# gusanagy/Hybrid-Diffusion-Underwater-Atmopheric-Image-Enhancement

Hardware: AMD Instinct MI355X
Metric: denoising-steps/sec (256x256, T=1000) (higher is better)
Workload: dtype f32 (tensors and accumulation fp32; every operand of the attention contractions as 2xfp16 pieces -- scores: a balance per product term, four terms at d_head 16 / three at d_head 32; P.V: three terms -- and of the 3x3 convs behind GroupNorm likewise (other 3x3 convs: 3xbf16 pieces), on the 16-bit MFM

## Files before the change

### hybrid-diffusion-underwater-atmopheric-image-enhancement_amd/csrc/conv1x1_x3.hip

```cpp
#include <stdlib.h>

#include "common.h"
#include "conv_x3.h"
#include "device.h"

using namespace hdiff;

namespace {

constexpr int THREADS = 256;

__device__ constexpr int TERM_W[6] = {2, 1, 0, 1, 0, 0};
__device__ constexpr int TERM_X[6] = {0, 1, 2, 0, 1, 0};

template <bool WLDS>
__global__ __launch_bounds__(THREADS, 3) void conv1x1_x3_kernel(const Conv1x1X3K p) {
  constexpr int MT = 2, WN = 2;
  __shared__ __attribute__((aligned(16))) u32x4 sW[WLDS ? 2 : 1][WLDS ? 3 * 64 * 2 : 1];
  const int tid = threadIdx.x, lane = tid & 63, wave = tid >> 6;
  const int l31 = lane & 31, h = lane >> 5;
  int cob = blockIdx.x, tile_id = blockIdx.y;
  if ((gridDim.y & 7u) == 0u && gridDim.x > 1u) {
    const unsigned lin = blockIdx.x + gridDim.x * blockIdx.y, per = 8u * gridDim.x;
    const unsigned grp = lin / per, r = lin - grp * per;
    tile_id = (int)(grp * 8u + (r & 7u));
    cob = (int)(r >> 3);
  }
  const int co0 = cob * 64;
  const long px0 = ((long)tile_id * 4 + __builtin_amdgcn_readfirstlane(wave)) * 64;
  const int b = blockIdx.z;
  const int C1 = p.Cin - p.C0;
  const unsigned hw = (unsigned)p.HW;
  const float* x0b = p.x0 + (size_t)b * p.C0 * p.HW + px0;
  const float* x1b = p.x1 ? p.x1 + (size_t)b * C1 * p.HW + px0 - (size_t)p.C0 * p.HW : x0b;
  const unsigned* wlane = p.wp3 + ((size_t)(co0 + l31) * 8 + h * 4);
  const size_t w_piece = (size_t)p.CoutPad * 8, w_chunk = 3 * w_piece;

  f32x16 acc[MT][WN];
#pragma unroll
  for (int mt = 0; mt < MT; ++mt)
#pragma unroll
    for (int nt = 0; nt < WN; ++nt)
#pragma unroll
      for (int r = 0; r < 16; ++r) acc[mt][nt][r] = 0.f;

  constexpr int XD = 1;
  const int nchunks = p.Cin / 16;
  f32x2 xr[XD + 1][8];
  u32x4 wr[2][MT][3];
  auto load_x = [&](f32x2 (&x)[8], int c) {
    c = min(c, nchunks - 1);
    const float* xb = (16 * c < p.C0) ? x0b : x1b;
    const unsigned k0 = (unsigned)(16 * c + 8 * h);
#pragma unroll
    for (int j = 0; j < 8; ++j) x[j] = *reinterpret_cast<const f32x2*>(xb + (size_t)((k0 + j) * hw + 2u * l31));
  };
  auto load_w = [&](u32x4 (&w)[MT][3], int c) {
    const unsigned* wb = wlane + (size_t)min(c, nchunks - 1) * w_chunk;
#pragma unroll
    for (int mt = 0; mt < MT; ++mt)
#pragma unroll
      for (int pc = 0; pc < 3; ++pc) w[mt][pc] = *reinterpret_cast<const u32x4*>(wb + pc * w_piece + (size_t)mt * 32 * 8);
  };
  auto mma = [&](const f32x2 (&x)[8], const u32x4 (&w)[MT][3]) {
    u32x4 xp[WN][3];
#pragma unroll
    for (int nt = 0; nt < WN; ++nt)
#pragma unroll
      for (int j = 0; j < 4; ++j) {
        unsigned h0, h1, h2;
        split3(x[2 * j][nt], x[2 * j + 1][nt], h0, h1, h2);
        xp[nt][0][j] = h0; xp[nt][1][j] = h1; xp[nt][2][j] = h2;
      }
#pragma unroll
    for (int t = 0; t < 6; ++t) {
      if ((HDIFF_MUTANT & 1) && TERM_W[t] == 0 && TERM_X[t] == 2) continue;
#pragma unroll
      for (int mt = 0; mt < MT; ++mt)
#pragma unroll
        for (int nt = 0; nt < WN; ++nt) acc[mt][nt] = mfma_bf16(w[mt][TERM_W[t]], xp[nt][TERM_X[t]], acc[mt][nt]);
    }
  };

  if constexpr (WLDS) {
    const unsigned* wsrc[2];
    int wdst[2];
#pragma unroll
    for (int i = 0; i < 2; ++i) {
      int u = i * THREADS + tid;
      if (u >= 384) u -= 128;
      const int pc = u >> 7, rem = u & 127;
      wsrc[i] = p.wp3 + (size_t)pc * w_piece + (size_t)(co0 + (rem >> 1)) * 8 + (rem & 1) * 4;
      wdst[i] = u;
    }
    u32x4 wst[2];
    auto wload = [&](int c) {
      const size_t off = (size_t)min(c, nchunks - 1) * w_chunk;
#pragma unroll
      for (int i = 0; i < 2; ++i) wst[i] = *reinterpret_cast<const u32x4*>(wsrc[i] + off);
    };
    auto wstore = [&](int buf) {
#pragma unroll
      for (int i = 0; i < 2; ++i) sW[buf][wdst[i]] = wst[i];
    };
    auto wread = [&](u32x4 (&w)[MT][3], int buf) {
#pragma unroll
      for (int mt = 0; mt < MT; ++mt)
#pragma unroll
        for (int pc = 0; pc < 3; ++pc) w[mt][pc] = sW[buf][(pc * 64 + 32 * mt + l31) * 2 + h];
    };
    wload(0);
    load_x(xr[0], 0);
    wstore(0);
    __syncthreads();
    for (int c = 0; c < nchunks; c += 2) {
#pragma unroll
      for (int i = 0; i < 2; ++i) {
        if (c + i < nchunks) {
          wload(c + i + 1);
          load_x(xr[(i + 1) & 1], c + i + 1);
          wread(wr[0], i);
          mma(xr[i], wr[0]);
          wstore((i + 1) & 1);
          asm volatile("s_waitcnt lgkmcnt(0)\n\ts_barrier" ::: "memory");
        }
      }
    }
  } else {
#pragma unroll
    for (int i = 0; i < XD; ++i) load_x(xr[i], i);
    load_w(wr[0], 0);
    for (int c = 0; c < nchunks; c += XD + 1) {
#pragma unroll
      for (int i = 0; i < XD + 1; ++i) {
        if (c + i < nchunks) {
          load_x(xr[(i + XD) % (XD + 1)], c + i + XD);
          load_w(wr[(i + 1) & 1], c + i + 1);
          mma(xr[i], wr[i & 1]);
        }
      }
    }
  }

  const size_t blk = ((size_t)b * p.Cout) * p.HW + px0;
  const bool full = co0 + 64 <= p.Cout;
  const bool track = p.absmax_out != nullptr;
  unsigned amax = 0u;
#pragma unroll
  for (int mt = 0; mt < MT; ++mt) {
#pragma unroll
    for (int r0 = 0; r0 < 16; r0 += 8) {
      f32x2 res[8];
      float add[8];
      bool ok[8];
#pragma unroll
      for (int j = 0; j < 8; ++j) {
        const int r = r0 + j;
        const int co = co0 + 32 * mt + (r & 3) + 8 * (r >> 2) + 4 * h;
        ok[j] = full || co < p.Cout;
        const int cc = ok[j] ? co : 0;
        float a = 0.f;
        if (p.bias) a += p.bias[cc];
        if (p.addvec) a += p.addvec[(size_t)b * p.Cout + cc];
        add[j] = a;
        if (p.residual) res[j] = *reinterpret_cast<const f32x2*>(p.residual + blk + (size_t)cc * p.HW + 2u * l31);
      }
#pragma unroll
      for (int j = 0; j < 8; ++j) {
        const int r = r0 + j;
        const int co = co0 + 32 * mt + (r & 3) + 8 * (r >> 2) + 4 * h;
        f32x2 v = {acc[mt][0][r], acc[mt][1][r]};
        v += add[j];
        if (p.residual) v += res[j];
        if (ok[j]) *reinterpret_cast<f32x2*>(p.out + blk + (size_t)co * p.HW + 2u * l31) = v;
        if (track && ok[j]) {
          const unsigned v0 = __builtin_bit_cast(unsigned, v[0]) & 0x7fffffffu, v1 = __builtin_bit_cast(unsigned, v[1]) & 0x7fffffffu;
          const unsigned vm = v0 > v1 ? v0 : v1;
          amax = vm > amax ? vm : amax;
        }
      }
    }
  }
  if (track) {
#pragma unroll
    for (int o = 32; o > 0; o >>= 1) {
      const unsigned other = (unsigned)__shfl_xor((int)amax, o, 64);
      amax = other > amax ? other : amax;
    }
    if (lane == 0) atomicMax(&p.absmax_out[b], amax);
  }
}

}

namespace hdiff {

void launch_conv1x1_x3(const Conv1x1X3K& k, int B, hipStream_t stream) {
  dim3 grid(cdiv(k.Cout, 64), (unsigned)(k.HW / 256), B);
  hipLaunchKernelGGL(conv1x1_x3_kernel<true>, grid, dim3(THREADS), 0, stream, k);
}

}
```

Baseline: 3.018.

## Add persistent LDS-resident-weight kernel for 1x1 x3 convolution

Adds a persistent kernel variant where each workgroup loads the whole 3-piece weight slice for its 64 output channels into LDS once, then loops over pixel tiles with cross-tile prefetch of the next input chunk and next bias/addvec. This is meant to remove repeated per-tile weight streaming and LDS double-buffer barriers, and to amortise launch and tail cost by sizing the grid to the device's CU count with XCD-aware slot mapping. It relies on large dynamic LDS (up to 160KB) and falls back to the old kernel when that cannot be set or occupancy would be poor.

Measured after the change: 3.024, median of 2. Within noise of the previous version (+0.2%).

```diff
diff --git a/hybrid-diffusion-underwater-atmopheric-image-enhancement_amd/csrc/conv1x1_x3.hip b/hybrid-diffusion-underwater-atmopheric-image-enhancement_amd/csrc/conv1x1_x3.hip
--- a/hybrid-diffusion-underwater-atmopheric-image-enhancement_amd/csrc/conv1x1_x3.hip
+++ b/hybrid-diffusion-underwater-atmopheric-image-enhancement_amd/csrc/conv1x1_x3.hip
@@ -1,4 +1,6 @@
 #include <stdlib.h>
+
+#include <atomic>
 
 #include "common.h"
 #include "conv_x3.h"
@@ -191,12 +193,237 @@
   }
 }
 
+#ifndef CONV1X1_RESIDENT
+#define CONV1X1_RESIDENT 1
+#endif
+constexpr int res_wps(bool res) { return res ? 2 : 3; }
+template <int NW, bool RES>
+__global__ __launch_bounds__(NW * 64, res_wps(RES)) void conv1x1_x3_resident_kernel(const Conv1x1X3K p, const int B, const int nslots) {
+  constexpr int MT = 2, WN = 2, NT = NW * 64;
+  extern __shared__ __attribute__((aligned(16))) u32x4 sWr[];
+  const int tid = threadIdx.x, lane = tid & 63, wave = __builtin_amdgcn_readfirstlane(tid >> 6);
+  const int l31 = lane & 31, h = lane >> 5;
+  const unsigned per = 8u * (gridDim.x / (unsigned)nslots);
+  const unsigned grp = blockIdx.x / per, r = blockIdx.x - grp * per;
+  const int slot = (int)(grp * 8u + (r & 7u)), co0_wg = (int)(r >> 3) * 64;
+  const int tps = (int)(p.HW >> 6), ntiles = B * tps, tstep = nslots * NW;
+  if (slot * NW >= ntiles) return;
+  const int C1 = p.Cin - p.C0;
+  const unsigned hw = (unsigned)p.HW;
+  const int nchunks = p.Cin / 16;
+  const size_t w_piece = (size_t)p.CoutPad * 8, w_chunk = 3 * w_piece;
+
+  const int nunits = nchunks * 384;
+  for (int u0 = tid; u0 < nunits; u0 += 4 * NT) {
+    u32x4 v[4];
+#pragma unroll
+    for (int i = 0; i < 4; ++i) {
+      const int u = min(u0 + i * NT, nunits - 1);
+      const int c = u / 384, q = u - c * 384, pc = q >> 7, rem = q & 127;
+      v[i] = *reinterpret_cast<const u32x4*>(p.wp3 + (size_t)c * w_chunk + (size_t)pc * w_piece + (size_t)(co0_wg + (rem >> 1)) * 8 + (rem & 1) * 4);
+    }
+#pragma unroll
+    for (int i = 0; i < 4; ++i)
+      if (u0 + i * NT < nunits) sWr[u0 + i * NT] = v[i];
+  }
+  __syncthreads();
+
+  struct Tile { const float* x0; const float* x1; int b; long px0; };
+  auto tile_at = [&](int t) {
+    const int b = t / tps;
+    const long px0 = (long)(t - b * tps) * 64;
+    const float* x0 = p.x0 + (size_t)b * p.C0 * p.HW + px0;
+    return Tile{x0, p.x1 ? p.x1 + (size_t)b * C1 * p.HW + px0 - (size_t)p.C0 * p.HW : x0, b, px0};
+  };
+  auto load_x = [&](f32x2 (&x)[8], const float* x0, const float* x1, int c) {
+    const float* xb = (16 * c < p.C0) ? x0 : x1;
+    const unsigned k0 = (unsigned)(16 * c + 8 * h);
+#pragma unroll
+    for (int j = 0; j < 8; ++j) x[j] = *reinterpret_cast<const f32x2*>(xb + (size_t)((k0 + j) * hw + 2u * l31));
+  };
+  f32x16 acc[MT][WN];
+  auto mma = [&](const f32x2 (&x)[8], int c) {
+    u32x4 w[MT][3];
+#pragma unroll
+    for (int mt = 0; mt < MT; ++mt)
+#pragma unroll
+      for (int pc = 0; pc < 3; ++pc) w[mt][pc] = sWr[c * 384 + (pc * 64 + 32 * mt + l31) * 2 + h];
+    u32x4 xp[WN][3];
+#pragma unroll
+    for (int nt = 0; nt < WN; ++nt)
+#pragma unroll
+      for (int j = 0; j < 4; ++j) {
+        unsigned h0, h1, h2;
+        split3(x[2 * j][nt], x[2 * j + 1][nt], h0, h1, h2);
+        xp[nt][0][j] = h0; xp[nt][1][j] = h1; xp[nt][2][j] = h2;
+      }
+#pragma unroll
+    for (int t = 0; t < 6; ++t) {
+      if ((HDIFF_MUTANT & 1) && TERM_W[t] == 0 && TERM_X[t] == 2) continue;
+#pragma unroll
+      for (int mt = 0; mt < MT; ++mt)
+#pragma unroll
+        for (int nt = 0; nt < WN; ++nt) acc[mt][nt] = mfma_bf16(w[mt][TERM_W[t]], xp[nt][TERM_X[t]], acc[mt][nt]);
+    }
+  };
+
+  const bool track = p.absmax_out != nullptr;
+  const int t0 = slot * NW + wave;
+  if (t0 >= ntiles) return;
+  auto row_of = [&](int g, int j) { const int q = (g & 1) * 8 + j; return 32 * (g >> 1) + (q & 3) + 8 * (q >> 2); };
+  const unsigned voff = ((unsigned)(4 * h) * hw + 2u * l31) * 4u;
+  auto addend_load = [&](int co0, int b, float& bl, float& al) {
+    const int cl = co0 + lane < p.Cout ? co0 + lane : 0;
+    bl = 0.f; al = 0.f;
+    if (p.bias) bl = p.bias[cl];
+    if (p.addvec) al = p.addvec[(size_t)b * p.Cout + cl];
+  };
+
+  auto run = [&](auto full_c) {
+    constexpr bool FULL = decltype(full_c)::value;
+    int t = t0;
+    Tile cur = tile_at(t);
+    f32x2 xr[2][8];
+    load_x(xr[0], cur.x0, cur.x1, 0);
+    float addl;
+    {
+      float bl, al;
+      addend_load(co0_wg, cur.b, bl, al);
+      addl = (0.f + bl) + al;
+    }
+    for (;;) {
+      const int tn = t + tstep;
+      const bool more = tn < ntiles;
+      const Tile nxt = tile_at(more ? tn : t);
+      int co0 = co0_wg;
+      asm volatile("" : "+s"(co0));
+#pragma unroll
+      for (int mt = 0; mt < MT; ++mt)
+#pragma unroll
+        for (int nt = 0; nt < WN; ++nt)
+#pragma unroll
+          for (int q = 0; q < 16; ++q) acc[mt][nt][q] = 0.f;
+      auto step = [&](f32x2 (&use)[8], f32x2 (&fill)[8], int c) {
+        const bool wrap = c + 1 == nchunks;
+        load_x(fill, wrap ? nxt.x0 : cur.x0, wrap ? nxt.x1 : cur.x1, wrap ? 0 : c + 1);
+        mma(use, c);
+      };
+      step(xr[0], xr[1], 0);
+      for (int c = 1; c < nchunks; c += 2) {
+        step(xr[1], xr[0], c);
+        if (c + 1 < nchunks) step(xr[0], xr[1], c + 1);
+      }
+
+      const int b = cur.b;
+      const size_t blk = ((size_t)b * p.Cout) * p.HW + cur.px0;
+      auto at = [&](const float* base, int g, int j) {
+        return reinterpret_cast<const char*>(base + blk + (size_t)(co0 + row_of(g, j)) * p.HW) + voff;
+      };
+      auto res_load = [&](f32x2 (&res)[8], int g) {
+#pragma unroll
+        for (int j = 0; j < 8; ++j)
+          if (FULL || co0 + row_of(g, j) + 4 * h < p.Cout) res[j] = *reinterpret_cast<const f32x2*>(at(p.residual, g, j));
+      };
+      float bl_n, al_n;
+      addend_load(co0, nxt.b, bl_n, al_n);
+      f32x2 res[2][8];
+      if constexpr (RES) res_load(res[0], 0);
+      unsigned amax = 0u, amax1 = 0u;
+#pragma unroll
+      for (int g = 0; g < 4; ++g) {
+        if constexpr (RES)
+          if (g + 1 < 4) res_load(res[(g + 1) & 1], g + 1);
+#pragma unroll
+        for (int j = 0; j < 8; ++j) {
+          const int q = (g & 1) * 8 + j, ch = row_of(g, j) + 4 * h;
+          const bool ok = FULL || co0 + ch < p.Cout;
+          const float add = __shfl(addl, ch, 64);
+          float p0 = acc[g >> 1][0][q] + add, p1 = acc[g >> 1][1][q] + add;
+          if constexpr (RES) { p0 += res[g & 1][j][0]; p1 += res[g & 1][j][1]; }
+          if (ok) *reinterpret_cast<f32x2*>(const_cast<char*>(at(p.out, g, j))) = f32x2{p0, p1};
+          if (track && ok) {
+            const unsigned v0 = __builtin_bit_cast(unsigned, p0) & 0x7fffffffu, v1 = __builtin_bit_cast(unsigned, p1) & 0x7fffffffu;
+            amax = v0 > amax ? v0 : amax;
+            amax1 = v1 > amax1 ? v1 : amax1;
+          }
+        }
+      }
+      if (track) {
+        amax = amax1 > amax ? amax1 : amax;
+#pragma unroll
+        for (int o = 32; o > 0; o >>= 1) {
+          const unsigned other = (unsigned)__shfl_xor((int)amax, o, 64);
+          amax = other > amax ? other : amax;
+        }
+        if (lane == 0) atomicMax(&p.absmax_out[b], amax);
+      }
+      if (!more) break;
+      float zero = 0.f;
+      asm volatile("" : "+v"(zero));
+      addl = (zero + bl_n) + al_n;
+      if (nchunks & 1) {
+#pragma unroll
+        for (int j = 0; j < 8; ++j) xr[0][j] = xr[1][j];
+      }
+      t = tn;
+      cur = nxt;
+    }
+  };
+  if (co0_wg + 64 <= p.Cout) run(std::true_type{});
+  else run(std::false_type{});
+}
+
+
+constexpr int RES_LDS_MAX = 160 * 1024;
+struct ResidentDev { int cus; bool big; };
+bool resident_dev(ResidentDev& out) {
+  constexpr int MAXDEV = 64;
+  static std::atomic<signed char> state[MAXDEV];
+  static ResidentDev known[MAXDEV];
+  int dev = -1;
+  if (hipGetDevice(&dev) != hipSuccess || dev < 0 || dev >= MAXDEV) return false;
+  if (state[dev].load(std::memory_order_acquire) == 0) {
+    ResidentDev d{0, false};
+    if (hipDeviceGetAttribute(&d.cus, hipDeviceAttributeMultiprocessorCount, dev) != hipSuccess) d.cus = 0;
+    d.big = hipFuncSetAttribute(reinterpret_cast<const void*>(&conv1x1_x3_resident_kernel<12, false>), hipFuncAttributeMaxDynamicSharedMemorySize,
+                                RES_LDS_MAX) == hipSuccess &&
+            hipFuncSetAttribute(reinterpret_cast<const void*>(&conv1x1_x3_resident_kernel<8, true>), hipFuncAttributeMaxDynamicSharedMemorySize,
+                                RES_LDS_MAX) == hipSuccess;
+    (void)hipGetLastError();
+    known[dev] = d;
+    state[dev].store(1, std::memory_order_release);
+  }
+  out = known[dev];
+  return out.cus >= 8;
+}
+
 }
 
 namespace hdiff {
 
 void launch_conv1x1_x3(const Conv1x1X3K& k, int B, hipStream_t stream) {
-  dim3 grid(cdiv(k.Cout, 64), (unsigned)(k.HW / 256), B);
+  const int ncb = cdiv(k.Cout, 64);
+  const int lds = k.Cin * 384;
+  ResidentDev dev;
+  if (CONV1X1_RESIDENT && lds <= RES_LDS_MAX && resident_dev(dev)) {
+    const bool res = k.residual != nullptr;
+    const bool small = lds <= 48 * 1024;
+    const int nw = small ? 4 : 4 * res_wps(res);
+    const int wg_xcd = (dev.cus / 8) * (small ? res_wps(res) : 1);
+    const int slots_xcd = wg_xcd / ncb;
+    const long wg_tiles = ((long)B * (k.HW / 64) + nw - 1) / nw;
+    if (slots_xcd * ncb * 8 >= wg_xcd * 7 && (small || dev.big)) {
+      const long want = (wg_tiles + 7) / 8 * 8;
+      const int nslots = (int)(want < 8L * slots_xcd ? want : 8L * slots_xcd);
+      const dim3 grid(nslots * ncb);
+      if (small && res) hipLaunchKernelGGL((conv1x1_x3_resident_kernel<4, true>), grid, dim3(256), lds, stream, k, B, nslots);
+      else if (small) hipLaunchKernelGGL((conv1x1_x3_resident_kernel<4, false>), grid, dim3(256), lds, stream, k, B, nslots);
+      else if (res) hipLaunchKernelGGL((conv1x1_x3_resident_kernel<8, true>), grid, dim3(512), lds, stream, k, B, nslots);
+      else hipLaunchKernelGGL((conv1x1_x3_resident_kernel<12, false>), grid, dim3(768), lds, stream, k, B, nslots);
+      return;
+    }
+  }
+  dim3 grid(ncb, (unsigned)(k.HW / 256), B);
   hipLaunchKernelGGL(conv1x1_x3_kernel<true>, grid, dim3(THREADS), 0, stream, k);
 }
 
```
